# algbio/GraphChainer

Hardware: AMD Instinct MI355X
Metric: reads_per_sec (higher is better)
Workload: dtype u64

## Files before the change

graphchainer_amd/csrc/batch/gc_batch_long.inc:

```
	void prepareWholeReadPass()
	{
		uint64_t nLongSeeds = 0;
		maxReadLen = 1;
		for (uint64_t r = 0; r < n; r++) maxReadLen = std::max<uint64_t>(maxReadLen, R->offsets[r + 1] - R->offsets[r]);
		firstAlnCap = (uint32_t)std::max<uint64_t>(32, maxReadLen / 512);
		if (sw.testLongMaxAlignments) firstAlnCap = *sw.testLongMaxAlignments;
		alnSlots = n * (uint64_t)firstAlnCap;
		if (P->long_pass && alnSlots >= 0xffffffffull) throw std::runtime_error("batch too large for the whole-read pass");
		if (P->long_pass) {
			nLongSeeds = nSeedsTotal;
			if (nLongSeeds >= 0xffffffffull) throw std::runtime_error("batch too large for the whole-read pass");
			hJobs = st->hLongJobs.reserve<LongJob>(n);
			cellPoolPinned = sw.testLongCellsPerBase || P->capacity.long_cells_per_base > 0;
			uint64_t cellsPerBase = (uint64_t)std::max<int64_t>(2, capacityOr(sw.testLongCellsPerBase, P->capacity.long_cells_per_base, (int64_t)st->longCellsPerBase));
			if (sw.testLongForceFallback && !cellPoolPinned) cellsPerBase *= 3;
			cellBudget = cellBudgetFor(cellsPerBase);
			pool.run(n, [&](size_t r, size_t) {
				const ReadGlue& gl = glue[r];
				LongJob& j = hJobs[r];
				j.maskOff = R->maskOff[r];
				j.maskWords = R->maskWords[r];
				j.alnCap = firstAlnCap;
				j.readOff = R->offsets[r];
				j.readLen = (uint32_t)(R->offsets[r + 1] - R->offsets[r]);
// ... 32 lines not shown
			syncStream(ls);
			dLongState = st->longState.reserve<LongState>(n);
			workCapacity = 8 * n + 64;
			dLongWork = st->longWork.reserve<LongWork>(workCapacity);
			dLongWorkResults = st->longWorkResults.reserve<LongWorkResult>(workCapacity);
			dCandSeed = st->longCandSeed.reserve<uint32_t>(2 * workCapacity);
			dWorkLen = st->longWorkLen.reserve<uint32_t>(workCapacity);
			dRetryList = st->longRetryList.reserve<uint32_t>(workCapacity);
			dOrder = st->longOrder.reserve<uint32_t>(workCapacity);
			roundTraceBudget = 0;
			for (uint64_t r = 0; r < n; r++) { uint64_t len = R->offsets[r + 1] - R->offsets[r]; roundTraceBudget += 4 * ((P->force_global || clip.on() ? 2 * len + 2 : len + len / 2) + 1024); }
			dRoundTrace = st->longRoundTrace.reserve<unsigned long long>(roundTraceBudget);
			uint64_t scratchBudget = P->capacity.long_scratch_bytes > 0 ? (uint64_t)P->capacity.long_scratch_bytes : (48ull << 30) / (uint64_t)longTokenCount(sw.longTokens, n, st->batchesDone, st->fragShare);
			if (sw.testLongScratchGb) scratchBudget = *sw.testLongScratchGb << 30;
			scratchLanes = std::min<uint64_t>(std::min<uint64_t>(workCapacity + 64, 2 * n + 128), std::max<uint64_t>(2048, std::min<uint64_t>(65536 + 64, scratchBudget / (waveWords * 8))));
			longScratchWords = scratchLanes * waveWords;
			shareLongScratch = sw.shareLongScratch();
			if (!shareLongScratch) dLongScratchOwn = st->longScratch.reserve<unsigned long long>(longScratchWords);
		}
	}

	uint64_t cellBudgetFor(uint64_t perBase) const { uint64_t b = 0; for (uint64_t r = 0; r < n; r++) b += perBase * (R->offsets[r + 1] - R->offsets[r]) + 1024; return b; }

	bool growLongCells()
	{
		bool overflowed = false;
		for (uint64_t r = 0; r < n && !overflowed; r++) overflowed = hLongResults[r].status == 4;
		if (!overflowed || cellPoolPinned) return false;
		HIP_CHECK(hipMemcpyAsync(hLongSmall, dLongCursor, sizeof(unsigned long long), hipMemcpyDeviceToHost, ls));
		syncStream(ls);
		const uint64_t asked = hLongSmall[0], bases = std::max<uint64_t>(1, R->totalBases);
		const uint64_t next = std::max<uint64_t>(st->longCellsPerBase + 2, (asked + asked / 2 + bases - 1) / bases);
		if (sw.debugTimes) fprintf(stderr, "[gc mem] the whole-read pass runs again: %.2f G merged-trace cells asked for, %.2f G reserved (%llu per read base), now %llu per base\n", asked / 1e9, cellBudget / 1e9, (unsigned long long)st->longCellsPerBase, (unsigned long long)next);
		if (next > 256 || cellBudgetFor(next) * sizeof(LongCell) > (64ull << 30)) return false;
		st->longCellsPerBase = next;
		cellBudget = cellBudgetFor(next);
		dLongCells = st->longCells.reserve<LongCell>(cellBudget, true);
		HIP_CHECK(hipMemsetAsync(dLongCursor, 0, cursorWords * sizeof(unsigned long long), ls));
		syncStream(ls);
		return true;
	}

	static constexpr uint32_t LONG_ALN_SLOTS_MAX = 1u << 16;
	bool growAlnSlots(const std::vector<uint32_t>& reads, bool keep)
	{
		uint64_t total = alnSlots;
		std::vector<std::pair<uint32_t, uint32_t>> grown;
		for (uint32_t r : reads) {
			const uint32_t cap = hJobs[r].alnCap, limit = std::min<uint32_t>(LONG_ALN_SLOTS_MAX, std::max<uint32_t>(1, hJobs[r].seedEnd - hJobs[r].seedBegin));
			if (cap >= limit) continue;
			const uint32_t next = (uint32_t)std::min<uint64_t>(limit, 4ull * cap);
			if (total + next >= 0xffffffffull) continue;
			grown.push_back({ r, next });
			total += next;
		}
		if (grown.empty()) return false;
		if (sw.debugTimes) fprintf(stderr, "[gc mem] %zu reads found more whole-read alignments than they had slots for and run again: %llu -> %llu slots in the batch\n", grown.size(), (unsigned long long)alnSlots, (unsigned long long)total);
		if (keep && total * sizeof(LongAln) > st->longAlns.bytes) {
// ... 24 lines not shown

	void runLongRounds()
	{
		if (n == 0) return;
		unsigned long long* dLongScratch = nullptr;
		hipStream_t q = ls;
		hipEvent_t* ring = nullptr;
		auto collect = [&](int slot) { float ms = 0; HIP_CHECK(hipEventElapsedTime(&ms, ring[2 * slot], ring[2 * slot + 1])); longExtendUs += (double)ms * 1000.0; };
		int timedRounds = 0;
		unsigned long long* cursor = dLongCursor + 32;
		volatile unsigned long long* hCursor = hLongSmall + 32;
		double dbgWaitUs = 0;
		const double dbgT0 = nowUs();
		launchLongInit(q, dLongJobs, (uint32_t)n, dLongState);
		uint32_t lastWork = 0xffffffffu;

		for (int round = 0; round < 4096; round++) {
			launchZeroWords(q, cursor, 4);
			uint32_t maxCand = 1;
			if (round > 0 && lastWork > 0) maxCand = (uint32_t)std::min<uint64_t>(8, std::max<uint64_t>(1, (2 * n) / lastWork));
			if (round > 0 && lastWork < 8192) maxCand = 8;
			if (round > 0 && lastWork > 0) maxCand = (uint32_t)std::min<uint64_t>(maxCand, std::max<uint64_t>(1, (8 * n) / lastWork));
			if (sw.testLongSpeculate) maxCand = *sw.testLongSpeculate;
			launchLongSelect(q, G->dev, dLongJobs, (uint32_t)n, dLongSeeds, R->totalBases, (uint32_t)P->min_cluster_size, (uint32_t)P->extra_heuristic, maxCand, dLongState, dLongAlns, dLongCells, dLongWork, dWorkLen, dCandSeed, cursor, workCapacity);
			launchLongOrder(q, dWorkLen, cursor, dOrder, (uint32_t)maxReadLen, sw.testLongOrder);
			launchPublish(q, cursor, (unsigned long long*)hCursor, 2);
			const double tWait0 = nowUs();
			syncStream(q);
			dbgWaitUs += nowUs() - tWait0;
			uint32_t nWorkItems = (uint32_t)hCursor[0];
			if (nWorkItems == 0) break;
			if (!dLongScratch) {
				longTokenTake();
				dLongScratch = shareLongScratch ? longScratchOfToken : dLongScratchOwn;
				q = passRounds->q;
				ring = passRounds->ring;
			}
			uint32_t team = longExtendTeamSize(nWorkItems, sw.testLongTeam.value_or(0));
			uint32_t blocks = std::min<uint32_t>((nWorkItems + team - 1) / team, (uint32_t)std::max<uint64_t>(1, (scratchLanes - 64) / team));
			if (sw.testLongMaxBlocks) blocks = std::min<uint32_t>(blocks, *sw.testLongMaxBlocks);
			if (timedRounds >= LONG_EVENT_RING) collect(timedRounds % LONG_EVENT_RING);
			hipEvent_t ev0 = ring[2 * (timedRounds % LONG_EVENT_RING)], ev1 = ring[2 * (timedRounds % LONG_EVENT_RING) + 1];
			HIP_CHECK(hipEventRecord(ev0, q));
			launchLongExtend(q, G->dev, G->devTables, R->devMasks, lcfg, dLongWork, dOrder, nWorkItems, dLongScratch, team, blocks,
				dRoundTrace, cursor + 1, roundTraceBudget, dLongWorkResults, dLongCursor + 8, cursor + 2, 0, nullptr, team == 1 ? dRetryList : nullptr, cursor + 3);
			if (team == 1) {
				if ((uint64_t)blocks * team < nWorkItems) launchZeroWords(q, cursor + 2, 1);
				uint32_t retryBlocks = std::min<uint32_t>(128, (uint32_t)std::max<uint64_t>(1, (scratchLanes - 64) / 2));
				launchLongExtend(q, G->dev, G->devTables, R->devMasks, lcfg, dLongWork, dRetryList, nWorkItems, dLongScratch, 2, retryBlocks,
					dRoundTrace, cursor + 1, roundTraceBudget, dLongWorkResults, dLongCursor + 8, cursor + 2, EXT_LDS_CAP, cursor + 3);
			}
			HIP_CHECK(hipEventRecord(ev1, q));
			launchLongMerge(q, G->dev, dLongJobs, (uint32_t)n, dLongSeeds, dCandSeed, dLongWorkResults, dRoundTrace, dLongState, dLongAlns, dLongCells, dLongCursor, cellBudget, (uint32_t)P->extra_heuristic);
			lastWork = nWorkItems;
			timedRounds++;
			longRounds++;
		}
		const double dbgT1 = nowUs();
		if (ring) for (int k = std::max(0, timedRounds - LONG_EVENT_RING); k < timedRounds; k++) collect(k % LONG_EVENT_RING);
		longTokenDrop();
		launchLongFinish(ls, (uint32_t)n, dLongState, hLongResults);
		syncStream(ls);
		if (sw.debugTimes) {
			const char* hwq = getenv("GPU_MAX_HW_QUEUES");
			fprintf(stderr, "[gc times] whole-read rounds: %.1f ms in all, %.1f ms waiting for the rounds' work counts, %.1f ms in the last wait, %d rounds, GPU_MAX_HW_QUEUES=%s\n", (nowUs() - dbgT0) / 1e3, dbgWaitUs / 1e3, (nowUs() - dbgT1) / 1e3, timedRounds, hwq ? hwq : "unset");
		}
	}

// ... 223 lines not shown
```

graphchainer_amd/csrc/hip/gc_kernels.hip:

```cpp
#include "gc_kernels.hpp"
#include "gc_device_wave.hpp"
#include <cstdlib>

namespace gcdev {


__device__ __forceinline__ int baseCode(uint8_t c)
{
	switch (c) {
		case 'a': case 'A': return 0;
		case 'c': case 'C': return 1;
		case 'g': case 'G': return 2;
		case 't': case 'T': return 3;
	}
	return -1;
}

__device__ __forceinline__ uint32_t hashKmer(uint64_t kmer)
{
	kmer *= 0x9E3779B97F4A7C15ull;
	return (uint32_t)(kmer >> 32);
}

__device__ __forceinline__ uint32_t filterBit(uint64_t kmer, uint32_t shift) { return (uint32_t)((kmer * 0xD6E8FEB86659FD93ull) >> shift); }
// ... 858 lines not shown
	for (uint32_t a = aFrom; a < aTo; a++)
		if (mine[a].start <= sd.seqPos && mine[a].end >= sd.seqPos && (extraHeuristic || mine[a].goodness > sd.goodness)) return 1;
	int32_t compareNode = g.nodeIDs[sd.node];
	uint32_t compareOffset = g.nodeOffset[sd.node] + sd.offset;
	for (uint32_t a = aFrom; a < aTo; a++) {
		int on = onTrace(cellPool + mine[a].traceOff, mine[a].traceLen, sd.seqPos, compareNode, compareOffset);
		if (on == 2) return 2;
		if (on == 1) return 1;
	}
	return 0;
}

#define LONG_MAX_CANDIDATES 8
__device__ __forceinline__ void longSelectRead(const DGraph& g, const uint32_t r, const uint32_t lane, const LongJob* __restrict__ jobs, const LongSeed* __restrict__ seeds, uint32_t minClusterSize,
	uint32_t extraHeuristic, uint32_t maxCandidates, LongState* __restrict__ state, const LongAln* __restrict__ alns, const LongCell* __restrict__ cellPool, LongWork* __restrict__ work, uint32_t* __restrict__ workLen, uint32_t* __restrict__ candSeed,
	unsigned long long* __restrict__ workCount, uint64_t workCapacity)
{
	LongState st = state[r];
	st.candCount = 0;
	if (st.status != 0) { if (lane == 0) state[r] = st; return; }
	LongJob job = jobs[r];
	const LongAln* mine = alns + job.alnBegin;
	uint32_t cand[LONG_MAX_CANDIDATES];
	uint32_t nCand = 0;
	uint32_t si = st.si;
	bool stop = false;
	while (!stop && si < job.seedEnd) {
		const uint32_t idx = si + lane;
		const bool valid = idx < job.seedEnd;
		LongSeed sd = seeds[valid ? idx : si];
		const bool cut = valid && (seedCutEndToEnd(sd.goodness, st.e2eScore, extraHeuristic)
// ... 9 lines not shown
		for (; b < limit; b++) {
			if ((assertMask >> b) & 1) { st.status = 1; stop = true; break; }
			if ((candMask >> b) & 1) {
				if (nCand > 0 && st.extended + nCand >= job.extendSeeds) { stop = true; break; }
				for (uint32_t k = 0; k < LONG_MAX_CANDIDATES; k++) if (k == nCand) cand[k] = si + b;
				nCand++;
				if (nCand == maxCandidates) { b++; stop = true; break; }
			}
		}
		si += b;
		if (!stop && firstCut < nValid) { si = job.seedEnd; stop = true; }
	}
	st.si = si;
	if (nCand > 0) {
		unsigned long long at = 0;
		if (lane == 0) at = atomicAdd(workCount, 2ull * nCand);
		at = __shfl(at, 0);
		if (at + 2ull * nCand > workCapacity) { st.status = 2; nCand = 0; }
		st.candBegin = (uint32_t)(at / 2);
		st.candCount = nCand;
		uint32_t myCand = 0;
		for (uint32_t k = 0; k < LONG_MAX_CANDIDATES; k++) if (k == lane) myCand = cand[k];
		if (lane < nCand) {
			const uint32_t c = lane;
			LongSeed sd = seeds[myCand];
			const uint32_t L = job.readLen, p = sd.seqPos;
			uint32_t twinNode, twinOffset;
			twinOf(g, sd.node, sd.offset, twinNode, twinOffset);
			work[at + 2 * c] = LongWork { job.maskOff + 4ull * job.maskWords, job.maskWords, L - p, p, twinNode, twinOffset, r };
			work[at + 2 * c + 1] = LongWork { job.maskOff, job.maskWords, p + 1, L - 1 - p, sd.node, sd.offset, r };
			workLen[at + 2 * c] = p;
			workLen[at + 2 * c + 1] = L - 1 - p;
			candSeed[at / 2 + c] = myCand;
		}
	}
	if (lane == 0) state[r] = st;
}
__global__ void __launch_bounds__(64) k_long_select(DGraph g, const LongJob* __restrict__ jobs, uint32_t nReads, const LongSeed* __restrict__ seeds, uint64_t rcBase, uint32_t minClusterSize,
	uint32_t extraHeuristic, uint32_t maxCandidates, LongState* __restrict__ state, const LongAln* __restrict__ alns, const LongCell* __restrict__ cellPool, LongWork* __restrict__ work, uint32_t* __restrict__ workLen, uint32_t* __restrict__ candSeed,
	unsigned long long* __restrict__ workCount, uint64_t workCapacity)
{
	GC_RAISE_PRIO();
	const uint32_t r = blockIdx.x, lane = threadIdx.x;
	if (r >= nReads) return;
	longSelectRead(g, r, lane, jobs, seeds, minClusterSize, extraHeuristic, maxCandidates, state, alns, cellPool, work, workLen, candSeed, workCount, workCapacity);
}

#ifndef GC_LONG_MIN_WAVES
#define GC_LONG_MIN_WAVES 1
#endif
template <int LANES, bool PERSISTENT, bool BAND = false, bool CLIP = false>
#ifndef GC_LONG_WAVES_ONE
#define GC_LONG_WAVES_ONE 5
#endif
__global__ void __launch_bounds__(64) __attribute__((amdgpu_waves_per_eu(LANES == 1 ? GC_LONG_WAVES_ONE : GC_LONG_MIN_WAVES, 8))) k_long_extend(DGraph g, const CorrectnessTables* __restrict__ ct, const uint64_t* __restrict__ masks, ExtendConfig cfg,
	const LongWork* __restrict__ work, const uint32_t* __restrict__ order, uint32_t nWork, unsigned long long* __restrict__ scratch, uint64_t wordsPerLane,
	unsigned long long* __restrict__ tracePool, unsigned long long* __restrict__ traceCursor, uint64_t traceCapacity, LongWorkResult* __restrict__ results, unsigned long long* __restrict__ counters,
	unsigned long long* __restrict__ nextSlot, uint32_t retryStatus, const unsigned long long* __restrict__ nWorkOnDevice, uint32_t* __restrict__ capListOut, unsigned long long* __restrict__ capCountOut)
{
	__shared__ WaveLdsT<LANES> lds;
// ... 25 lines not shown
		const uint32_t w = order[slot];
		if (retryStatus != 0 && results[w].status != retryStatus) { if (PERSISTENT) continue; else break; }
		LongWork it = work[w];
		LongWorkResult res { 0, 0, EXT_FAILED, 0, 0 };
		if (it.seqLen > 0) {
			uint32_t nTrace = 0;
			int32_t score = 0;
			EqSource eqSrc { masks + it.maskOff, it.maskWords, it.startBit };
			if (CLIP) res.status = extendSeedWave<LANES == 1, true, true>(g, *ct, eqSrc, cfg.bandwidth, (lds_u32*)&lds.w[0][0], wsx, (int)it.seqLen, it.node, it.offset, 0, nTrace, score, cnt,
				cfg.rampBandwidth, cfg.maxCells, cfg.forceGlobal != 0, cfg.clipErrorCost(), cfg.xDrop);
			else if (BAND) res.status = extendSeedWave<LANES == 1, true>(g, *ct, eqSrc, cfg.bandwidth, (lds_u32*)&lds.w[0][0], wsx, (int)it.seqLen, it.node, it.offset, 0, nTrace, score, cnt,
				cfg.rampBandwidth, cfg.maxCells, cfg.forceGlobal != 0);
			else res.status = extendSeedWave<LANES == 1>(g, *ct, eqSrc, cfg.bandwidth, (lds_u32*)&lds.w[0][0], wsx, (int)it.seqLen, it.node, it.offset, 0, nTrace, score, cnt);
			res.score = score;
			res.pad = cnt.flattenTie;
			if (res.status == EXT_OK) {
				unsigned long long base = 0;
				if (leader) base = atomicAdd(traceCursor, (unsigned long long)nTrace);
				if (LANES == 1) base = (unsigned long long)__builtin_amdgcn_readfirstlane((uint32_t)base) | ((unsigned long long)__builtin_amdgcn_readfirstlane((uint32_t)(base >> 32)) << 32);
				if (base + nTrace <= traceCapacity) {
					if (LANES == 1) { for (uint32_t i = threadIdx.x; i < nTrace; i += 64) tracePool[base + i] = wsx.word(wsx.traceBase(i, 0)); }
					else for (uint32_t i = 0; i < nTrace; i++) tracePool[base + i] = wsx.word(wsx.traceBase(i, 0));
					res.traceOff = base;
					res.traceLen = nTrace;
				} else res.status = EXT_OVERFLOW;
			}
		}
		if (leader) results[w] = res;
		if (leader && capListOut && res.status == EXT_LDS_CAP) capListOut[atomicAdd(capCountOut, 1ull)] = w;
	}
	if (cnt.extensions && leader) {
		atomicAdd(&counters[0], cnt.dpTiles);
		atomicAdd(&counters[1], cnt.recomputeTiles);
		atomicAdd(&counters[2], cnt.columnSteps);
		atomicAdd(&counters[3], cnt.traceItems);
		atomicAdd(&counters[4], cnt.extensions);
		atomicAdd(&counters[5], cnt.backtraceTiles);
#ifdef GC_STAMPS
		for (int i = 0; i < 16; i++) atomicAdd(&counters[8 + i], cnt.cyc[i]);
#endif
	}
}

__device__ __forceinline__ void longMergeRead(const DGraph& g, const uint32_t r, const uint32_t lane, const LongJob* __restrict__ jobs, const LongSeed* __restrict__ seeds, const uint32_t* __restrict__ candSeed,
	const LongWorkResult* __restrict__ results, const unsigned long long* __restrict__ tracePool,
	LongState* state, LongAln* alns, LongCell* cellPool, unsigned long long* __restrict__ cellCursor, uint64_t cellCapacity, uint32_t extraHeuristic)
{
	LongState st = state[r];
	if (st.candCount == 0 || st.status != 0) return;
	LongJob job = jobs[r];
	LongAln* mine = alns + job.alnBegin;
	const int L = (int)job.readLen;
	const uint32_t nAlnAtSelect = st.nAln;
	for (uint32_t c = 0; c < st.candCount && st.status == 0; c++) {
		const uint32_t pair = st.candBegin + c;
		const uint32_t seedIdx = candSeed[pair];
		LongSeed sd = seeds[seedIdx];
		if (c > 0) {
			if (seedCutEndToEnd(sd.goodness, st.e2eScore, extraHeuristic)) { st.si = job.seedEnd; break; }
			if (seedCutBudget(sd.goodness, st.extended, job.extendSeeds, st.worstExtended, extraHeuristic)) { st.si = job.seedEnd; break; }
// ... 11 lines not shown
		if (runF && stB != EXT_ASSERT) st.pad1 += rf.pad & 1u;
		if (stB == EXT_ASSERT || stF == EXT_ASSERT) { st.status = 1; break; }
		if (stB == EXT_OVERFLOW || stF == EXT_OVERFLOW) { st.status = 2; break; }
		if (stB == EXT_LDS_CAP || stF == EXT_LDS_CAP) { st.status = 5; break; }
		bool hasB = stB == EXT_OK, hasF = stF == EXT_OK;
		if (!hasB && !hasF) continue;
		uint32_t nB = rb.traceLen, nF = rf.traceLen;
		uint32_t useB = hasB ? (hasF ? nB - 1 : nB) : 0;
		uint32_t total = useB + (hasF ? nF : 0);
		if (st.nAln >= job.alnCap) { st.status = 3; break; }
		unsigned long long base = 0;
		if (lane == 0) base = atomicAdd(cellCursor, (unsigned long long)total);
		base = __shfl(base, 0);
		if (base + total > cellCapacity) { st.status = 4; break; }
		LongCell* outCells = cellPool + base;
		for (uint32_t i = lane; i < useB; i += 64) {
			TraceCell tc = unpackCell(tracePool[rb.traceOff + i]);
			uint32_t off = tc.offsetAndSwitch & 255u;
			int32_t id = g.nodeIDs[tc.node];
			uint32_t orig = g.nodeOffset[tc.node] + off;
			LongCell oc;
			oc.node = id ^ 1;
			oc.offset = g.origSize[id] - 1 - orig;
			oc.seqPos = (uint32_t)(p - 1 - tc.seqPos);
			oc.nodeSwitch = (i + 1 < nB) ? ((unpackCell(tracePool[rb.traceOff + i + 1]).offsetAndSwitch >> 8) & 1u) : 0u;
			outCells[i] = oc;
		}
		if (hasF) for (uint32_t i = lane; i < nF; i += 64) {
			TraceCell tc = unpackCell(tracePool[rf.traceOff + (nF - 1 - i)]);
			LongCell oc;
			oc.node = g.nodeIDs[tc.node];
			oc.offset = g.nodeOffset[tc.node] + (tc.offsetAndSwitch & 255u);
			oc.seqPos = (uint32_t)(p + 1 + tc.seqPos);
			oc.nodeSwitch = (tc.offsetAndSwitch >> 8) & 1u;
			outCells[useB + i] = oc;
		}
		__threadfence_block();
		LongAln al;
		al.start = outCells[0].seqPos;
		al.end = outCells[total - 1].seqPos + 1;
		al.score = (uint32_t)((hasB ? rb.score : 0) + (hasF ? rf.score : 0));
		al.goodness = sd.goodness;
		al.traceOff = base;
		al.traceLen = total;
		al.pad = 0;
		uint32_t e2e = 0;
		if (lane == 0) {
			mine[st.nAln] = al;
			e2e = endToEndScore(mine, st.nAln + 1, (uint32_t)L, st.e2eScore);
		}
		st.nAln++;
		st.e2eScore = __shfl(e2e, 0);
		__threadfence_block();
	}
	st.candCount = 0;
	if (lane == 0) state[r] = st;
}

__global__ void __launch_bounds__(64) k_long_merge(DGraph g, const LongJob* __restrict__ jobs, uint32_t nReads, const LongSeed* __restrict__ seeds, const uint32_t* __restrict__ candSeed,
	const LongWorkResult* __restrict__ results, const unsigned long long* __restrict__ tracePool,
	LongState* state, LongAln* alns, LongCell* cellPool, unsigned long long* __restrict__ cellCursor, uint64_t cellCapacity, uint32_t extraHeuristic)
{
	GC_RAISE_PRIO();
	const uint32_t r = blockIdx.x;
	if (r >= nReads) return;
	longMergeRead(g, r, threadIdx.x, jobs, seeds, candSeed, results, tracePool, state, alns, cellPool, cellCursor, cellCapacity, extraHeuristic);
}

#ifndef GC_ORDER_THREADS
#define GC_ORDER_THREADS 256
#endif
__global__ void __launch_bounds__(GC_ORDER_THREADS) k_long_order(const uint32_t* __restrict__ workLen, const unsigned long long* __restrict__ workCount, uint32_t* __restrict__ order, uint32_t shift, uint32_t mode)
{
	GC_RAISE_PRIO();
	__shared__ uint32_t hist[1024];
	__shared__ uint32_t start[1024];
	const uint32_t n = (uint32_t)*workCount, tid = threadIdx.x, T = GC_ORDER_THREADS;
	if (mode == 0) { for (uint32_t i = tid; i < n; i += T) order[i] = i; return; }
	for (uint32_t b = tid; b < 1024; b += T) hist[b] = 0;
	__syncthreads();
	for (uint32_t i = tid; i < n; i += T) { uint32_t b = workLen[i] >> shift; atomicAdd(&hist[1023 - (b < 1023 ? b : 1023)], 1u); }
// ... 102 lines not shown
	const bool small = caps.capAnchors <= CHAIN_LDS_ANCHORS / 2 && caps.capTable <= CHAIN_LDS_WIDTH / 2;
	if (!ldsLaunch) {}
	else if (small) hipLaunchKernelGGL(HIP_KERNEL_NAME(k_chain<2>), dim3(chainGridBlocks(nReads)), dim3(64), 0, stream, g, jobs, nReads, anchors, frags, fragStatus, splitLen, splitGap, caps, scratch, chainScratchBytes(caps), chainOut, chainLen, chainScore, chainStatus, forceScratch ? 1u : 0u);
	else hipLaunchKernelGGL(HIP_KERNEL_NAME(k_chain<1>), dim3(chainGridBlocks(nReads)), dim3(64), 0, stream, g, jobs, nReads, anchors, frags, fragStatus, splitLen, splitGap, caps, scratch, chainScratchBytes(caps), chainOut, chainLen, chainScore, chainStatus, forceScratch ? 1u : 0u);
	const bool cannotBeNeeded = !forceScratch && caps.capAnchors <= CHAIN_LDS_ANCHORS / (small ? 2 : 1) && caps.capEndpoints <= CHAIN_LDS_ENTRIES / (small ? 2 : 1) && caps.capTable <= CHAIN_LDS_WIDTH / (small ? 2 : 1);
	hipLaunchKernelGGL(HIP_KERNEL_NAME(k_chain<0>), dim3(cannotBeNeeded ? (nReads < 64 ? nReads : 64) : chainScratchBlocks(nReads)), dim3(64), 0, stream, g, jobs, nReads, anchors, frags, fragStatus, splitLen, splitGap, caps, scratch, chainScratchBytes(caps), chainOut, chainLen, chainScore, chainStatus, scratchFlags);
}

uint64_t longWaveWordsPerLane(const ExtendConfig& cfg) { return waveScratchWords(cfg.maxSlices, cfg.maxItems, cfg.maxTrace, cfg.maxCols); }

void launchLongInit(hipStream_t stream, const LongJob* jobs, uint32_t nReads, LongState* state)
{
	if (nReads) hipLaunchKernelGGL(k_long_init, dim3((nReads + 255) / 256), dim3(256), 0, stream, jobs, nReads, state);
}
void launchLongSelect(hipStream_t stream, const DGraph& g, const LongJob* jobs, uint32_t nReads, const LongSeed* seeds, uint64_t rcBase, uint32_t minClusterSize, uint32_t extraHeuristic, uint32_t maxCandidates,
	LongState* state, const LongAln* alns, const LongCell* cellPool, LongWork* work, uint32_t* workLen, uint32_t* candSeed, unsigned long long* workCount, uint64_t workCapacity)
{
	if (maxCandidates < 1) maxCandidates = 1;
	if (maxCandidates > LONG_MAX_CANDIDATES) maxCandidates = LONG_MAX_CANDIDATES;
	if (nReads) hipLaunchKernelGGL(k_long_select, dim3(nReads), dim3(64), 0, stream, g, jobs, nReads, seeds, rcBase, minClusterSize, extraHeuristic, maxCandidates, state, alns, cellPool, work, workLen, candSeed, workCount, workCapacity);
}
uint32_t longExtendTeamSize(uint32_t nWork, uint32_t teamOverride)
{
	if (teamOverride) return teamOverride;
	(void)nWork;
	return 1;
}

void launchLongExtend(hipStream_t stream, const DGraph& g, const CorrectnessTables* ct, const uint64_t* masks, const ExtendConfig& cfg, const LongWork* work, const uint32_t* order, uint32_t nWork,
	unsigned long long* scratch, uint32_t lanes, uint32_t blocks, unsigned long long* tracePool, unsigned long long* traceCursor, uint64_t traceCapacity, LongWorkResult* results, unsigned long long* counters,
	unsigned long long* nextSlot, uint32_t retryStatus, const unsigned long long* nWorkOnDevice, uint32_t* capListOut, unsigned long long* capCountOut)
{
	if (!nWork) return;
	uint64_t words = longWaveWordsPerLane(cfg);
	const bool persistent = nWorkOnDevice || (uint64_t)blocks * lanes < nWork;
	const bool band = cfg.bandControls();
	const bool clip = cfg.clipOn();
#define GC_LAUNCH_ONE(N, P, B, C) hipLaunchKernelGGL(HIP_KERNEL_NAME(k_long_extend<N, P, B, C>), dim3(blocks), dim3(64), 0, stream, g, ct, masks, cfg, work, order, nWork, scratch, words, tracePool, traceCursor, traceCapacity, results, counters, nextSlot, retryStatus, nWorkOnDevice, capListOut, capCountOut)
#define GC_LAUNCH_TEAM(N) do { if (clip) { if (persistent) GC_LAUNCH_ONE(N, true, true, true); else GC_LAUNCH_ONE(N, false, true, true); } \
	else if (band) { if (persistent) GC_LAUNCH_ONE(N, true, true, false); else GC_LAUNCH_ONE(N, false, true, false); } \
	else if (persistent) GC_LAUNCH_ONE(N, true, false, false); else GC_LAUNCH_ONE(N, false, false, false); } while (0)
	switch (lanes) {
		case 1: GC_LAUNCH_TEAM(1); break;
		case 2: GC_LAUNCH_TEAM(2); break;
		case 4: GC_LAUNCH_TEAM(4); break;
		case 8: GC_LAUNCH_TEAM(8); break;
		case 16: GC_LAUNCH_TEAM(16); break;
		case 32: GC_LAUNCH_TEAM(32); break;
		default: GC_LAUNCH_TEAM(64); break;
	}
// ... 26 lines not shown
		f.pad = fr.read;
		work[2 * (size_t)slot] = b;
		work[2 * (size_t)slot + 1] = f;
		if (results) {
			results[2 * (size_t)slot] = ExtResult { 0, 0, EXT_NOT_RUN, 0, 0 };
			results[2 * (size_t)slot + 1] = ExtResult { 0, 0, EXT_NOT_RUN, 0, 0 };
		}
	}
}
void launchBuildFragmentWork(hipStream_t stream, const DGraph& g, const Fragment* frags, const uint32_t* fragFirstSeed, uint32_t nFrags, const FragSeed* readSeeds, const uint64_t* readOffsets,
	uint64_t totalBases, uint32_t splitLen, FragSeed* fragSeeds, ExtItem* work, ExtResult* results)
{
	if (nFrags) hipLaunchKernelGGL(k_build_fragment_work, dim3((nFrags + 255) / 256), dim3(256), 0, stream, g, frags, fragFirstSeed, nFrags, readSeeds, readOffsets, totalBases, splitLen, fragSeeds, work, results);
}
void launchLongMerge(hipStream_t stream, const DGraph& g, const LongJob* jobs, uint32_t nReads, const LongSeed* seeds, const uint32_t* candSeed, const LongWorkResult* results,
	const unsigned long long* tracePool, LongState* state, LongAln* alns, LongCell* cellPool, unsigned long long* cellCursor, uint64_t cellCapacity, uint32_t extraHeuristic)
{
	if (nReads) hipLaunchKernelGGL(k_long_merge, dim3(nReads), dim3(64), 0, stream, g, jobs, nReads, seeds, candSeed, results, tracePool, state, alns, cellPool, cellCursor, cellCapacity, extraHeuristic);
}
void launchLongOrder(hipStream_t stream, const uint32_t* workLen, const unsigned long long* workCount, uint32_t* order, uint32_t maxLen, uint32_t mode)
{
	uint32_t shift = 0;
	while ((maxLen >> shift) > 1023) shift++;
	hipLaunchKernelGGL(k_long_order, dim3(1), dim3(GC_ORDER_THREADS), 0, stream, workLen, workCount, order, shift, mode);
}
void launchPublish(hipStream_t stream, const unsigned long long* src, unsigned long long* dst, uint32_t nWords)
{
	hipLaunchKernelGGL(k_publish, dim3(1), dim3(64), 0, stream, src, dst, nWords);
}
void launchZeroWords(hipStream_t stream, unsigned long long* dst, uint32_t nWords)
{
	hipLaunchKernelGGL(k_zero_words, dim3(1), dim3(64), 0, stream, dst, nWords);
}
// ... 36 lines not shown
```

graphchainer_amd/csrc/hip/gc_kernels.hpp:

```cpp
#pragma once
#include "gc_device.hpp"

#ifndef GC_HELPER_PRIO
#define GC_HELPER_PRIO 3
#endif
#if GC_HELPER_PRIO
#define GC_RAISE_PRIO() __builtin_amdgcn_s_setprio(GC_HELPER_PRIO)
#else
#define GC_RAISE_PRIO() ((void)0)
#endif
#ifndef GC_ED_PRIO
#define GC_ED_PRIO 0
#endif
#if GC_ED_PRIO
#define GC_RAISE_ED_PRIO() __builtin_amdgcn_s_setprio(GC_ED_PRIO)
#else
#define GC_RAISE_ED_PRIO() ((void)0)
#endif

namespace gcdev {

struct StreamDrain { hipStream_t q; ~StreamDrain() { (void)hipStreamSynchronize(q); } };

struct SeedIndex {
// ... 110 lines not shown
	uint64_t traceOff;
	uint32_t traceLen;
	uint32_t pad;
};

struct LongReadResult { uint32_t nAlignments, seedsExtended, status, pad; };

struct LongState { uint32_t si, nAln, extended, status, e2eScore, candBegin, candCount, pad1, worstExtended, pad2; };
struct LongWork {
	uint64_t maskOff;
	uint32_t maskWords, startBit;
	uint32_t seqLen, node, offset;
	uint32_t read;
};
struct LongWorkResult { uint64_t traceOff; uint32_t traceLen, status; int32_t score; uint32_t pad; };

void launchSeedLookup(hipStream_t stream, const SeedIndex& idx, const char* bases, const uint64_t* readOff, uint32_t nReads,
	uint64_t* matchCursor, uint32_t* readMatchOff, uint32_t* readMatchCount, uint2* matches, uint64_t matchCapacity, uint32_t* tmp, uint64_t totalBases, const uint32_t* chunkRead, const uint64_t* packed, const uint64_t* invalid);

void launchSeedCaps(hipStream_t stream, const SeedIndex& idx, uint32_t nReads, const uint8_t* invalidRead, const uint2* matches, const uint32_t* readMatchOff, const uint32_t* readMatchCount,
	uint32_t* readSeedCap, uint32_t* readSeedOff, unsigned long long* total);
void launchSeedGlue(hipStream_t stream, const SeedIndex& idx, const DGraph& g, const uint64_t* readOff, uint32_t nReads, const uint8_t* invalidRead, const uint2* matches, const uint32_t* readMatchOff,
	const uint32_t* readMatchCount, const uint32_t* readSeedOff, const uint32_t* winCapOff, double density, uint32_t splitLen, uint32_t splitGap, bool longPass, const GlueStaging& st,
	uint32_t* perRead , LongSeed* longSeeds, FragSeed* readSeeds, Fragment* frags, uint32_t* fragFirstSeed, ReadChainJob* jobs, GlueRead* out, unsigned long long* cursors, bool forceGlobal = false);
uint64_t glueElemBytes();
struct SeedHit;
struct SeedLookup;
struct SeedHitArrays { uint32_t *node, *offset, *seqPos, *matchLen, *raw; };
void launchSeedResolve(hipStream_t stream, const SeedLookup& lookup, const SeedHit* hits, uint64_t nHits, const uint32_t* readHitOff, uint32_t nReads, const uint64_t* readOff, const SeedHitArrays& out,
	unsigned long long* firstBad);
// ... 46 lines not shown
uint64_t chainScratchBytes(const ChainCaps& caps);
uint32_t chainGridBlocks(uint32_t nReads);
uint32_t chainScratchBlocks(uint32_t nReads);
bool chainLdsLaunch(uint32_t fewestSlots, bool forceScratch);
void launchChain(hipStream_t stream, const DGraph& g, const ReadChainJob* jobs, uint32_t nReads, const AnchorRec* anchors, const Fragment* frags, const uint32_t* fragStatus,
	int32_t splitLen, int32_t splitGap, ChainCaps caps, uint8_t* scratch, uint32_t* chainOut, uint32_t* chainLen, unsigned long long* chainScore, uint32_t* chainStatus, bool plainScan, bool forceScratch = false,
	uint32_t fewestSlots = 0);

void launchLongPass(hipStream_t stream, const DGraph& g, const CorrectnessTables* ct, const uint8_t* iupac, const ExtendConfig& cfg, const LongJob* jobs, uint32_t nReads,
	const LongSeed* seeds, const char* bases, uint64_t rcBase, uint32_t minClusterSize, uint32_t extraHeuristic, uint8_t* scratch, uint64_t slabBytes,
	LongCell* cellPool, unsigned long long* cellCursor, uint64_t cellCapacity, LongAln* alns, LongReadResult* results, unsigned long long* counters);
uint64_t longSlabBytes(const ExtendConfig& cfg);
uint64_t longWaveWordsPerLane(const ExtendConfig& cfg);
void launchLongInit(hipStream_t stream, const LongJob* jobs, uint32_t nReads, LongState* state);
void launchLongSelect(hipStream_t stream, const DGraph& g, const LongJob* jobs, uint32_t nReads, const LongSeed* seeds, uint64_t rcBase, uint32_t minClusterSize, uint32_t extraHeuristic, uint32_t maxCandidates,
	LongState* state, const LongAln* alns, const LongCell* cellPool, LongWork* work, uint32_t* workLen, uint32_t* candSeed, unsigned long long* workCount, uint64_t workCapacity);
uint32_t longExtendTeamSize(uint32_t nWork, uint32_t teamOverride);
void launchLongExtend(hipStream_t stream, const DGraph& g, const CorrectnessTables* ct, const uint64_t* masks, const ExtendConfig& cfg, const LongWork* work, const uint32_t* order, uint32_t nWork,
	unsigned long long* scratch, uint32_t lanes, uint32_t blocks, unsigned long long* tracePool, unsigned long long* traceCursor, uint64_t traceCapacity, LongWorkResult* results, unsigned long long* counters,
	unsigned long long* nextSlot, uint32_t retryStatus = 0, const unsigned long long* nWorkOnDevice = nullptr, uint32_t* capListOut = nullptr, unsigned long long* capCountOut = nullptr);
void launchLongMerge(hipStream_t stream, const DGraph& g, const LongJob* jobs, uint32_t nReads, const LongSeed* seeds, const uint32_t* candSeed, const LongWorkResult* results,
	const unsigned long long* tracePool, LongState* state, LongAln* alns, LongCell* cellPool, unsigned long long* cellCursor, uint64_t cellCapacity, uint32_t extraHeuristic);
struct PathSeqJob {
	uint64_t srcOff;
	uint64_t outOff;
	uint32_t count;
	uint32_t outCap;
	uint32_t firstOffset, lastOffset;
};
struct EdRead { uint64_t readOff, eqOff; uint32_t len, words; };
struct EdPair {
	uint64_t lettersOff;
	uint32_t m;
	uint32_t lenIndex;
	uint32_t read;
	uint32_t k;
};
// ... 91 lines not shown
```

Measured before the change: 85250.

## Compact active reads across long-pass rounds and keep extend traces in scratch

```diff
diff --git a/graphchainer_amd/csrc/batch/gc_batch_long.inc b/graphchainer_amd/csrc/batch/gc_batch_long.inc
--- a/graphchainer_amd/csrc/batch/gc_batch_long.inc
+++ b/graphchainer_amd/csrc/batch/gc_batch_long.inc
@@ -70,7 +70,8 @@
 			uint64_t scratchBudget = P->capacity.long_scratch_bytes > 0 ? (uint64_t)P->capacity.long_scratch_bytes : (48ull << 30) / (uint64_t)longTokenCount(sw.longTokens, n, st->batchesDone, st->fragShare);
 			if (sw.testLongScratchGb) scratchBudget = *sw.testLongScratchGb << 30;
 			scratchLanes = std::min<uint64_t>(std::min<uint64_t>(workCapacity + 64, 2 * n + 128), std::max<uint64_t>(2048, std::min<uint64_t>(65536 + 64, scratchBudget / (waveWords * 8))));
-			longScratchWords = scratchLanes * waveWords;
+			const uint64_t budgetLanes = scratchBudget / (waveWords * 8);
+			longScratchWords = (scratchLanes + (budgetLanes > scratchLanes ? std::min<uint64_t>(LONG_RETRY_SLOTS, budgetLanes - scratchLanes) : 0)) * waveWords;
 			shareLongScratch = sw.shareLongScratch();
 			if (!shareLongScratch) dLongScratchOwn = st->longScratch.reserve<unsigned long long>(longScratchWords);
 		}
@@ -98,6 +99,7 @@
 	}
 
 	static constexpr uint32_t LONG_ALN_SLOTS_MAX = 1u << 16;
+	static constexpr uint64_t LONG_RETRY_SLOTS = 256;
 	bool growAlnSlots(const std::vector<uint32_t>& reads, bool keep)
 	{
 		uint64_t total = alnSlots;
@@ -152,6 +154,9 @@
 		const double dbgT0 = nowUs();
 		launchLongInit(q, dLongJobs, (uint32_t)n, dLongState);
 		uint32_t lastWork = 0xffffffffu;
+		uint32_t* const dActive[2] = { dCandSeed + workCapacity, dCandSeed + workCapacity + n };
+		uint32_t nActive = 0;
+		const uint64_t scratchSlots = longScratchWords / waveWords;
 
 		for (int round = 0; round < 4096; round++) {
 			launchZeroWords(q, cursor, 4);
@@ -160,7 +165,8 @@
 			if (round > 0 && lastWork < 8192) maxCand = 8;
 			if (round > 0 && lastWork > 0) maxCand = (uint32_t)std::min<uint64_t>(maxCand, std::max<uint64_t>(1, (8 * n) / lastWork));
 			if (sw.testLongSpeculate) maxCand = *sw.testLongSpeculate;
-			launchLongSelect(q, G->dev, dLongJobs, (uint32_t)n, dLongSeeds, R->totalBases, (uint32_t)P->min_cluster_size, (uint32_t)P->extra_heuristic, maxCand, dLongState, dLongAlns, dLongCells, dLongWork, dWorkLen, dCandSeed, cursor, workCapacity);
+			launchLongSelect(q, G->dev, dLongJobs, (uint32_t)n, dLongSeeds, R->totalBases, (uint32_t)P->min_cluster_size, (uint32_t)P->extra_heuristic, maxCand, dLongState, dLongAlns, dLongCells, dLongWork, dWorkLen, dCandSeed, cursor, workCapacity,
+				round > 0 ? dActive[(round - 1) & 1] : nullptr, nActive, dActive[round & 1]);
 			launchLongOrder(q, dWorkLen, cursor, dOrder, (uint32_t)maxReadLen, sw.testLongOrder);
 			launchPublish(q, cursor, (unsigned long long*)hCursor, 2);
 			const double tWait0 = nowUs();
@@ -168,6 +174,7 @@
 			dbgWaitUs += nowUs() - tWait0;
 			uint32_t nWorkItems = (uint32_t)hCursor[0];
 			if (nWorkItems == 0) break;
+			nActive = (uint32_t)(hCursor[0] >> 32);
 			if (!dLongScratch) {
 				longTokenTake();
 				dLongScratch = shareLongScratch ? longScratchOfToken : dLongScratchOwn;
@@ -180,16 +187,18 @@
 			if (timedRounds >= LONG_EVENT_RING) collect(timedRounds % LONG_EVENT_RING);
 			hipEvent_t ev0 = ring[2 * (timedRounds % LONG_EVENT_RING)], ev1 = ring[2 * (timedRounds % LONG_EVENT_RING) + 1];
 			HIP_CHECK(hipEventRecord(ev0, q));
+			const bool tracesStay = team == 1 && blocks >= nWorkItems;
 			launchLongExtend(q, G->dev, G->devTables, R->devMasks, lcfg, dLongWork, dOrder, nWorkItems, dLongScratch, team, blocks,
-				dRoundTrace, cursor + 1, roundTraceBudget, dLongWorkResults, dLongCursor + 8, cursor + 2, 0, nullptr, team == 1 ? dRetryList : nullptr, cursor + 3);
+				tracesStay ? nullptr : dRoundTrace, cursor + 1, roundTraceBudget, dLongWorkResults, dLongCursor + 8, cursor + 2, 0, nullptr, team == 1 ? dRetryList : nullptr, cursor + 3);
 			if (team == 1) {
 				if ((uint64_t)blocks * team < nWorkItems) launchZeroWords(q, cursor + 2, 1);
-				uint32_t retryBlocks = std::min<uint32_t>(128, (uint32_t)std::max<uint64_t>(1, (scratchLanes - 64) / 2));
-				launchLongExtend(q, G->dev, G->devTables, R->devMasks, lcfg, dLongWork, dRetryList, nWorkItems, dLongScratch, 2, retryBlocks,
+				const uint64_t retryFirst = tracesStay ? blocks : 0, retryRoom = tracesStay ? scratchSlots - blocks : scratchLanes - 64;
+				uint32_t retryBlocks = std::min<uint32_t>(128, (uint32_t)std::max<uint64_t>(1, retryRoom / 2));
+				launchLongExtend(q, G->dev, G->devTables, R->devMasks, lcfg, dLongWork, dRetryList, nWorkItems, dLongScratch + retryFirst * waveWords, 2, retryBlocks,
 					dRoundTrace, cursor + 1, roundTraceBudget, dLongWorkResults, dLongCursor + 8, cursor + 2, EXT_LDS_CAP, cursor + 3);
 			}
 			HIP_CHECK(hipEventRecord(ev1, q));
-			launchLongMerge(q, G->dev, dLongJobs, (uint32_t)n, dLongSeeds, dCandSeed, dLongWorkResults, dRoundTrace, dLongState, dLongAlns, dLongCells, dLongCursor, cellBudget, (uint32_t)P->extra_heuristic);
+			launchLongMerge(q, G->dev, dLongJobs, (uint32_t)n, dLongSeeds, dCandSeed, dLongWorkResults, dRoundTrace, dLongScratch, dActive[round & 1], nActive, dLongState, dLongAlns, dLongCells, dLongCursor, cellBudget, (uint32_t)P->extra_heuristic);
 			lastWork = nWorkItems;
 			timedRounds++;
 			longRounds++;
diff --git a/graphchainer_amd/csrc/hip/gc_kernels.hip b/graphchainer_amd/csrc/hip/gc_kernels.hip
--- a/graphchainer_amd/csrc/hip/gc_kernels.hip
+++ b/graphchainer_amd/csrc/hip/gc_kernels.hip
@@ -896,7 +896,7 @@
 #define LONG_MAX_CANDIDATES 8
 __device__ __forceinline__ void longSelectRead(const DGraph& g, const uint32_t r, const uint32_t lane, const LongJob* __restrict__ jobs, const LongSeed* __restrict__ seeds, uint32_t minClusterSize,
 	uint32_t extraHeuristic, uint32_t maxCandidates, LongState* __restrict__ state, const LongAln* __restrict__ alns, const LongCell* __restrict__ cellPool, LongWork* __restrict__ work, uint32_t* __restrict__ workLen, uint32_t* __restrict__ candSeed,
-	unsigned long long* __restrict__ workCount, uint64_t workCapacity)
+	unsigned long long* __restrict__ workCount, uint64_t workCapacity, uint32_t* __restrict__ activeOut)
 {
 	LongState st = state[r];
 	st.candCount = 0;
@@ -936,8 +936,10 @@
 	st.si = si;
 	if (nCand > 0) {
 		unsigned long long at = 0;
-		if (lane == 0) at = atomicAdd(workCount, 2ull * nCand);
+		if (lane == 0) at = atomicAdd(workCount, 2ull * nCand + (1ull << 32));
 		at = __shfl(at, 0);
+		const uint32_t listAt = (uint32_t)(at >> 32);
+		at &= 0xffffffffull;
 		if (at + 2ull * nCand > workCapacity) { st.status = 2; nCand = 0; }
 		st.candBegin = (uint32_t)(at / 2);
 		st.candCount = nCand;
@@ -955,17 +957,18 @@
 			workLen[at + 2 * c + 1] = L - 1 - p;
 			candSeed[at / 2 + c] = myCand;
 		}
+		if (lane == 0) activeOut[listAt] = r;
 	}
 	if (lane == 0) state[r] = st;
 }
 __global__ void __launch_bounds__(64) k_long_select(DGraph g, const LongJob* __restrict__ jobs, uint32_t nReads, const LongSeed* __restrict__ seeds, uint64_t rcBase, uint32_t minClusterSize,
 	uint32_t extraHeuristic, uint32_t maxCandidates, LongState* __restrict__ state, const LongAln* __restrict__ alns, const LongCell* __restrict__ cellPool, LongWork* __restrict__ work, uint32_t* __restrict__ workLen, uint32_t* __restrict__ candSeed,
-	unsigned long long* __restrict__ workCount, uint64_t workCapacity)
+	unsigned long long* __restrict__ workCount, uint64_t workCapacity, const uint32_t* __restrict__ activeIn, uint32_t* __restrict__ activeOut)
 {
 	GC_RAISE_PRIO();
-	const uint32_t r = blockIdx.x, lane = threadIdx.x;
+	const uint32_t r = activeIn ? activeIn[blockIdx.x] : blockIdx.x, lane = threadIdx.x;
 	if (r >= nReads) return;
-	longSelectRead(g, r, lane, jobs, seeds, minClusterSize, extraHeuristic, maxCandidates, state, alns, cellPool, work, workLen, candSeed, workCount, workCapacity);
+	longSelectRead(g, r, lane, jobs, seeds, minClusterSize, extraHeuristic, maxCandidates, state, alns, cellPool, work, workLen, candSeed, workCount, workCapacity, activeOut);
 }
 
 #ifndef GC_LONG_MIN_WAVES
@@ -1021,13 +1024,23 @@
 			else res.status = extendSeedWave<LANES == 1>(g, *ct, eqSrc, cfg.bandwidth, (lds_u32*)&lds.w[0][0], wsx, (int)it.seqLen, it.node, it.offset, 0, nTrace, score, cnt);
 			res.score = score;
 			res.pad = cnt.flattenTie;
-			if (res.status == EXT_OK) {
+			if (res.status == EXT_OK && LANES == 1 && !PERSISTENT && !tracePool) {
+				res.traceOff = (uint64_t)blockIdx.x * wordsPerLane + wsx.traceBase(0, 0);
+				res.traceLen = nTrace;
+				res.pad |= LONG_TRACE_IN_SCRATCH;
+			} else if (res.status == EXT_OK) {
 				unsigned long long base = 0;
 				if (leader) base = atomicAdd(traceCursor, (unsigned long long)nTrace);
 				if (LANES == 1) base = (unsigned long long)__builtin_amdgcn_readfirstlane((uint32_t)base) | ((unsigned long long)__builtin_amdgcn_readfirstlane((uint32_t)(base >> 32)) << 32);
 				if (base + nTrace <= traceCapacity) {
-					if (LANES == 1) { for (uint32_t i = threadIdx.x; i < nTrace; i += 64) tracePool[base + i] = wsx.word(wsx.traceBase(i, 0)); }
-					else for (uint32_t i = 0; i < nTrace; i++) tracePool[base + i] = wsx.word(wsx.traceBase(i, 0));
+					const uint32_t step = LANES == 1 ? 64u : 1u, last = nTrace ? nTrace - 1 : 0;
+					for (uint32_t i = LANES == 1 ? threadIdx.x : 0u; i < nTrace; i += 4 * step) {
+						unsigned long long v[4];
+#pragma unroll
+						for (uint32_t k = 0; k < 4; k++) { const uint32_t t = i + k * step; v[k] = wsx.word(wsx.traceBase(t < last ? t : last, 0)); }
+#pragma unroll
+						for (uint32_t k = 0; k < 4; k++) { const uint32_t t = i + k * step; if (t < nTrace) tracePool[base + t] = v[k]; }
+					}
 					res.traceOff = base;
 					res.traceLen = nTrace;
 				} else res.status = EXT_OVERFLOW;
@@ -1049,8 +1062,74 @@
 	}
 }
 
+#define LONG_MERGE_CHUNKS 4
+template <bool FULL> __device__ __forceinline__ void longCellsBackwardTrip(const DGraph& g, const unsigned long long* __restrict__ src, uint32_t nB, uint32_t useB, int p, LongCell* __restrict__ out, uint32_t lane, uint32_t i0)
+{
+	const uint32_t last = nB - 1;
+	unsigned long long w[LONG_MERGE_CHUNKS], sw[LONG_MERGE_CHUNKS + 1];
+#pragma unroll
+	for (uint32_t k = 0; k < LONG_MERGE_CHUNKS; k++) { const uint32_t t = i0 + 64 * k + lane; w[k] = src[t < last ? t : last]; }
+	const uint32_t tNext = i0 + 64 * LONG_MERGE_CHUNKS;
+	const unsigned long long wNext = src[tNext < last ? tNext : last];
+	int32_t id[LONG_MERGE_CHUNKS];
+	uint32_t nodeOff[LONG_MERGE_CHUNKS], size[LONG_MERGE_CHUNKS];
+#pragma unroll
+	for (uint32_t k = 0; k < LONG_MERGE_CHUNKS; k++) { id[k] = gcK(g.nodeIDs + (uint32_t)w[k]); nodeOff[k] = gcK(g.nodeOffset + (uint32_t)w[k]); }
+#pragma unroll
+	for (uint32_t k = 0; k < LONG_MERGE_CHUNKS; k++) size[k] = gcK(g.origSize + id[k]);
+#pragma unroll
+	for (uint32_t k = 0; k < LONG_MERGE_CHUNKS; k++) sw[k] = __ballot((w[k] >> 62) & 1u);
+	sw[LONG_MERGE_CHUNKS] = (wNext >> 62) & 1u;
+#pragma unroll
+	for (uint32_t k = 0; k < LONG_MERGE_CHUNKS; k++) {
+		const uint32_t t = i0 + 64 * k + lane;
+		const TraceCell tc = unpackCell(w[k]);
+		const uint32_t next = lane < 63 ? (uint32_t)(sw[k] >> (lane + 1)) & 1u : (uint32_t)sw[k + 1] & 1u;
+		LongCell oc;
+		oc.node = id[k] ^ 1;
+		oc.offset = size[k] - 1 - (nodeOff[k] + (tc.offsetAndSwitch & 255u));
+		oc.seqPos = (uint32_t)(p - 1 - tc.seqPos);
+		oc.nodeSwitch = t + 1 < nB ? next : 0u;
+		if (FULL || t < useB) out[t] = oc;
+	}
+}
+__device__ __forceinline__ void longCellsBackward(const DGraph& g, const unsigned long long* __restrict__ src, uint32_t nB, uint32_t useB, int p, LongCell* __restrict__ out, uint32_t lane)
+{
+	uint32_t i0 = 0;
+	for (; i0 + 64 * LONG_MERGE_CHUNKS <= useB; i0 += 64 * LONG_MERGE_CHUNKS) longCellsBackwardTrip<true>(g, src, nB, useB, p, out, lane, i0);
+	for (; i0 < useB; i0 += 64 * LONG_MERGE_CHUNKS) longCellsBackwardTrip<false>(g, src, nB, useB, p, out, lane, i0);
+}
+template <bool FULL> __device__ __forceinline__ void longCellsForwardTrip(const DGraph& g, const unsigned long long* __restrict__ src, uint32_t nF, int p, LongCell* __restrict__ out, uint32_t lane, uint32_t i0)
+{
+	const uint32_t last = nF - 1;
+	unsigned long long w[LONG_MERGE_CHUNKS];
+#pragma unroll
+	for (uint32_t k = 0; k < LONG_MERGE_CHUNKS; k++) { const uint32_t t = i0 + 64 * k + lane; w[k] = src[last - (t < last ? t : last)]; }
+	int32_t id[LONG_MERGE_CHUNKS];
+	uint32_t nodeOff[LONG_MERGE_CHUNKS];
+#pragma unroll
+	for (uint32_t k = 0; k < LONG_MERGE_CHUNKS; k++) { id[k] = gcK(g.nodeIDs + (uint32_t)w[k]); nodeOff[k] = gcK(g.nodeOffset + (uint32_t)w[k]); }
+#pragma unroll
+	for (uint32_t k = 0; k < LONG_MERGE_CHUNKS; k++) {
+		const uint32_t t = i0 + 64 * k + lane;
+		const TraceCell tc = unpackCell(w[k]);
+		LongCell oc;
+		oc.node = id[k];
+		oc.offset = nodeOff[k] + (tc.offsetAndSwitch & 255u);
+		oc.seqPos = (uint32_t)(p + 1 + tc.seqPos);
+		oc.nodeSwitch = (tc.offsetAndSwitch >> 8) & 1u;
+		if (FULL || t < nF) out[t] = oc;
+	}
+}
+__device__ __forceinline__ void longCellsForward(const DGraph& g, const unsigned long long* __restrict__ src, uint32_t nF, int p, LongCell* __restrict__ out, uint32_t lane)
+{
+	uint32_t i0 = 0;
+	for (; i0 + 64 * LONG_MERGE_CHUNKS <= nF; i0 += 64 * LONG_MERGE_CHUNKS) longCellsForwardTrip<true>(g, src, nF, p, out, lane, i0);
+	for (; i0 < nF; i0 += 64 * LONG_MERGE_CHUNKS) longCellsForwardTrip<false>(g, src, nF, p, out, lane, i0);
+}
+
 __device__ __forceinline__ void longMergeRead(const DGraph& g, const uint32_t r, const uint32_t lane, const LongJob* __restrict__ jobs, const LongSeed* __restrict__ seeds, const uint32_t* __restrict__ candSeed,
-	const LongWorkResult* __restrict__ results, const unsigned long long* __restrict__ tracePool,
+	const LongWorkResult* __restrict__ results, const unsigned long long* __restrict__ tracePool, const unsigned long long* __restrict__ scratch,
 	LongState* state, LongAln* alns, LongCell* cellPool, unsigned long long* __restrict__ cellCursor, uint64_t cellCapacity, uint32_t extraHeuristic)
 {
 	LongState st = state[r];
@@ -1092,27 +1171,8 @@
 		base = __shfl(base, 0);
 		if (base + total > cellCapacity) { st.status = 4; break; }
 		LongCell* outCells = cellPool + base;
-		for (uint32_t i = lane; i < useB; i += 64) {
-			TraceCell tc = unpackCell(tracePool[rb.traceOff + i]);
-			uint32_t off = tc.offsetAndSwitch & 255u;
-			int32_t id = g.nodeIDs[tc.node];
-			uint32_t orig = g.nodeOffset[tc.node] + off;
-			LongCell oc;
-			oc.node = id ^ 1;
-			oc.offset = g.origSize[id] - 1 - orig;
-			oc.seqPos = (uint32_t)(p - 1 - tc.seqPos);
-			oc.nodeSwitch = (i + 1 < nB) ? ((unpackCell(tracePool[rb.traceOff + i + 1]).offsetAndSwitch >> 8) & 1u) : 0u;
-			outCells[i] = oc;
-		}
-		if (hasF) for (uint32_t i = lane; i < nF; i += 64) {
-			TraceCell tc = unpackCell(tracePool[rf.traceOff + (nF - 1 - i)]);
-			LongCell oc;
-			oc.node = g.nodeIDs[tc.node];
-			oc.offset = g.nodeOffset[tc.node] + (tc.offsetAndSwitch & 255u);
-			oc.seqPos = (uint32_t)(p + 1 + tc.seqPos);
-			oc.nodeSwitch = (tc.offsetAndSwitch >> 8) & 1u;
-			outCells[useB + i] = oc;
-		}
+		if (useB) longCellsBackward(g, ((rb.pad & LONG_TRACE_IN_SCRATCH) ? scratch : tracePool) + rb.traceOff, nB, useB, p, outCells, lane);
+		if (hasF && nF) longCellsForward(g, ((rf.pad & LONG_TRACE_IN_SCRATCH) ? scratch : tracePool) + rf.traceOff, nF, p, outCells + useB, lane);
 		__threadfence_block();
 		LongAln al;
 		al.start = outCells[0].seqPos;
@@ -1136,13 +1196,13 @@
 }
 
 __global__ void __launch_bounds__(64) k_long_merge(DGraph g, const LongJob* __restrict__ jobs, uint32_t nReads, const LongSeed* __restrict__ seeds, const uint32_t* __restrict__ candSeed,
-	const LongWorkResult* __restrict__ results, const unsigned long long* __restrict__ tracePool,
+	const LongWorkResult* __restrict__ results, const unsigned long long* __restrict__ tracePool, const unsigned long long* __restrict__ scratch, const uint32_t* __restrict__ activeReads,
 	LongState* state, LongAln* alns, LongCell* cellPool, unsigned long long* __restrict__ cellCursor, uint64_t cellCapacity, uint32_t extraHeuristic)
 {
 	GC_RAISE_PRIO();
-	const uint32_t r = blockIdx.x;
+	const uint32_t r = activeReads[blockIdx.x];
 	if (r >= nReads) return;
-	longMergeRead(g, r, threadIdx.x, jobs, seeds, candSeed, results, tracePool, state, alns, cellPool, cellCursor, cellCapacity, extraHeuristic);
+	longMergeRead(g, r, threadIdx.x, jobs, seeds, candSeed, results, tracePool, scratch, state, alns, cellPool, cellCursor, cellCapacity, extraHeuristic);
 }
 
 #ifndef GC_ORDER_THREADS
@@ -1275,11 +1335,13 @@
 	if (nReads) hipLaunchKernelGGL(k_long_init, dim3((nReads + 255) / 256), dim3(256), 0, stream, jobs, nReads, state);
 }
 void launchLongSelect(hipStream_t stream, const DGraph& g, const LongJob* jobs, uint32_t nReads, const LongSeed* seeds, uint64_t rcBase, uint32_t minClusterSize, uint32_t extraHeuristic, uint32_t maxCandidates,
-	LongState* state, const LongAln* alns, const LongCell* cellPool, LongWork* work, uint32_t* workLen, uint32_t* candSeed, unsigned long long* workCount, uint64_t workCapacity)
+	LongState* state, const LongAln* alns, const LongCell* cellPool, LongWork* work, uint32_t* workLen, uint32_t* candSeed, unsigned long long* workCount, uint64_t workCapacity,
+	const uint32_t* activeIn, uint32_t nActiveIn, uint32_t* activeOut)
 {
 	if (maxCandidates < 1) maxCandidates = 1;
 	if (maxCandidates > LONG_MAX_CANDIDATES) maxCandidates = LONG_MAX_CANDIDATES;
-	if (nReads) hipLaunchKernelGGL(k_long_select, dim3(nReads), dim3(64), 0, stream, g, jobs, nReads, seeds, rcBase, minClusterSize, extraHeuristic, maxCandidates, state, alns, cellPool, work, workLen, candSeed, workCount, workCapacity);
+	const uint32_t waves = activeIn ? nActiveIn : nReads;
+	if (waves) hipLaunchKernelGGL(k_long_select, dim3(waves), dim3(64), 0, stream, g, jobs, nReads, seeds, rcBase, minClusterSize, extraHeuristic, maxCandidates, state, alns, cellPool, work, workLen, candSeed, workCount, workCapacity, activeIn, activeOut);
 }
 uint32_t longExtendTeamSize(uint32_t nWork, uint32_t teamOverride)
 {
@@ -1295,6 +1357,7 @@
 	if (!nWork) return;
 	uint64_t words = longWaveWordsPerLane(cfg);
 	const bool persistent = nWorkOnDevice || (uint64_t)blocks * lanes < nWork;
+	if (!tracePool && (persistent || lanes != 1)) throw std::logic_error("launchLongExtend: a trace can only stay in a slot that one lane of one work item owns");
 	const bool band = cfg.bandControls();
 	const bool clip = cfg.clipOn();
 #define GC_LAUNCH_ONE(N, P, B, C) hipLaunchKernelGGL(HIP_KERNEL_NAME(k_long_extend<N, P, B, C>), dim3(blocks), dim3(64), 0, stream, g, ct, masks, cfg, work, order, nWork, scratch, words, tracePool, traceCursor, traceCapacity, results, counters, nextSlot, retryStatus, nWorkOnDevice, capListOut, capCountOut)
@@ -1351,9 +1414,9 @@
 	if (nFrags) hipLaunchKernelGGL(k_build_fragment_work, dim3((nFrags + 255) / 256), dim3(256), 0, stream, g, frags, fragFirstSeed, nFrags, readSeeds, readOffsets, totalBases, splitLen, fragSeeds, work, results);
 }
 void launchLongMerge(hipStream_t stream, const DGraph& g, const LongJob* jobs, uint32_t nReads, const LongSeed* seeds, const uint32_t* candSeed, const LongWorkResult* results,
-	const unsigned long long* tracePool, LongState* state, LongAln* alns, LongCell* cellPool, unsigned long long* cellCursor, uint64_t cellCapacity, uint32_t extraHeuristic)
-{
-	if (nReads) hipLaunchKernelGGL(k_long_merge, dim3(nReads), dim3(64), 0, stream, g, jobs, nReads, seeds, candSeed, results, tracePool, state, alns, cellPool, cellCursor, cellCapacity, extraHeuristic);
+	const unsigned long long* tracePool, const unsigned long long* scratch, const uint32_t* activeReads, uint32_t nActive, LongState* state, LongAln* alns, LongCell* cellPool, unsigned long long* cellCursor, uint64_t cellCapacity, uint32_t extraHeuristic)
+{
+	if (nActive) hipLaunchKernelGGL(k_long_merge, dim3(nActive), dim3(64), 0, stream, g, jobs, nReads, seeds, candSeed, results, tracePool, scratch, activeReads, state, alns, cellPool, cellCursor, cellCapacity, extraHeuristic);
 }
 void launchLongOrder(hipStream_t stream, const uint32_t* workLen, const unsigned long long* workCount, uint32_t* order, uint32_t maxLen, uint32_t mode)
 {
diff --git a/graphchainer_amd/csrc/hip/gc_kernels.hpp b/graphchainer_amd/csrc/hip/gc_kernels.hpp
--- a/graphchainer_amd/csrc/hip/gc_kernels.hpp
+++ b/graphchainer_amd/csrc/hip/gc_kernels.hpp
@@ -148,6 +148,7 @@
 	uint32_t read;
 };
 struct LongWorkResult { uint64_t traceOff; uint32_t traceLen, status; int32_t score; uint32_t pad; };
+enum : uint32_t { LONG_TRACE_IN_SCRATCH = 2u };
 
 void launchSeedLookup(hipStream_t stream, const SeedIndex& idx, const char* bases, const uint64_t* readOff, uint32_t nReads,
 	uint64_t* matchCursor, uint32_t* readMatchOff, uint32_t* readMatchCount, uint2* matches, uint64_t matchCapacity, uint32_t* tmp, uint64_t totalBases, const uint32_t* chunkRead, const uint64_t* packed, const uint64_t* invalid);
@@ -224,13 +225,14 @@
 uint64_t longWaveWordsPerLane(const ExtendConfig& cfg);
 void launchLongInit(hipStream_t stream, const LongJob* jobs, uint32_t nReads, LongState* state);
 void launchLongSelect(hipStream_t stream, const DGraph& g, const LongJob* jobs, uint32_t nReads, const LongSeed* seeds, uint64_t rcBase, uint32_t minClusterSize, uint32_t extraHeuristic, uint32_t maxCandidates,
-	LongState* state, const LongAln* alns, const LongCell* cellPool, LongWork* work, uint32_t* workLen, uint32_t* candSeed, unsigned long long* workCount, uint64_t workCapacity);
+	LongState* state, const LongAln* alns, const LongCell* cellPool, LongWork* work, uint32_t* workLen, uint32_t* candSeed, unsigned long long* workCount, uint64_t workCapacity,
+	const uint32_t* activeIn, uint32_t nActiveIn, uint32_t* activeOut);
 uint32_t longExtendTeamSize(uint32_t nWork, uint32_t teamOverride);
 void launchLongExtend(hipStream_t stream, const DGraph& g, const CorrectnessTables* ct, const uint64_t* masks, const ExtendConfig& cfg, const LongWork* work, const uint32_t* order, uint32_t nWork,
 	unsigned long long* scratch, uint32_t lanes, uint32_t blocks, unsigned long long* tracePool, unsigned long long* traceCursor, uint64_t traceCapacity, LongWorkResult* results, unsigned long long* counters,
 	unsigned long long* nextSlot, uint32_t retryStatus = 0, const unsigned long long* nWorkOnDevice = nullptr, uint32_t* capListOut = nullptr, unsigned long long* capCountOut = nullptr);
 void launchLongMerge(hipStream_t stream, const DGraph& g, const LongJob* jobs, uint32_t nReads, const LongSeed* seeds, const uint32_t* candSeed, const LongWorkResult* results,
-	const unsigned long long* tracePool, LongState* state, LongAln* alns, LongCell* cellPool, unsigned long long* cellCursor, uint64_t cellCapacity, uint32_t extraHeuristic);
+	const unsigned long long* tracePool, const unsigned long long* scratch, const uint32_t* activeReads, uint32_t nActive, LongState* state, LongAln* alns, LongCell* cellPool, unsigned long long* cellCursor, uint64_t cellCapacity, uint32_t extraHeuristic);
 struct PathSeqJob {
 	uint64_t srcOff;
 	uint64_t outOff;
```

Result: no change. 84910 (-0.4%).
